# hby1320/pytorch_object_detection

Measured on AMD Instinct MI355X. Metric: images/sec HISFCOS-R50 640x640 inference, higher is better.
Workload: dtype f32

## Files before the change

pytorch_object_detection_amd/csrc/fd_conv_b2b.hip:

```cpp
#include "fd_conv_common.h"

struct B2BArgs {
    const float* x; const float* res; float* y; float* z;
    const float* scale1; const float* shift1; const float* scale2; const float* shift2;
    int x_cs, x_co, res_cs, res_co, y_cs, y_co, z_cs, z_co;
    int M, KT1, NT1, N2, act1, act2;
    unsigned x_bytes, y_bytes, z_bytes, res_bytes;
};

template <int TM, int TN2>
__global__ __launch_bounds__(64, 2) void conv1x1_b2b_kernel(B2BArgs a, const float* __restrict__ wf1_, const float* __restrict__ wf2_) {
    extern __shared__ __attribute__((aligned(16))) char smem[];
    float* As = reinterpret_cast<float*>(smem);
    float* A2 = As + 32 * TM * 32;
    constexpr int NL = 4 * TM;
    const int lane = threadIdx.x, l31 = lane & 31, lh = lane >> 5;
    const int m0 = blockIdx.x * 32 * TM;

    constexpr unsigned OOB = 0xC0000000u;
    const __amdgpu_buffer_rsrc_t xrsrc = __builtin_amdgcn_make_buffer_rsrc((void*)a.x, (short)0, (int)a.x_bytes, 0x00020000);
    const int lrow = lane >> 3, chunk = lane & 7;
    unsigned a_off[NL];
#pragma unroll
    for (int i = 0; i < NL; ++i) {
        const int m = m0 + lrow + 8 * i;
        a_off[i] = (m < a.M) ? ((unsigned)m * (unsigned)a.x_cs + (unsigned)(a.x_co + chunk * 4)) * 4u : OOB;
    }
    const float4* __restrict__ wf1 = reinterpret_cast<const float4*>(wf1_) + lane;
    const float4* __restrict__ wf2 = reinterpret_cast<const float4*>(wf2_) + lane;
    const int KT1 = a.KT1, KT2 = 2 * a.NT1;

    float4 ra[NL];
    auto load_a = [&](int kt) {
        const unsigned kb = (unsigned)kt * 128u;
#pragma unroll
        for (int i = 0; i < NL; ++i)
            ra[i] = __builtin_bit_cast(float4, __builtin_amdgcn_raw_buffer_load_b128(xrsrc, (int)(a_off[i] + kb), 0, 0));
    };
    auto store_a = [&]() {
#pragma unroll
        for (int i = 0; i < NL; ++i) *reinterpret_cast<float4*>(As + lds_off(lrow + 8 * i, chunk)) = ra[i];
    };

    f32x16 acc2[TM][TN2];
#pragma unroll
    for (int i = 0; i < TM; ++i)
#pragma unroll
        for (int j = 0; j < TN2; ++j)
#pragma unroll
            for (int e = 0; e < 16; ++e) acc2[i][j][e] = 0.f;

    const int c4 = (lane & 7) * 4, prow = lane >> 3;
    float* stage = As;
    const __amdgpu_buffer_rsrc_t yrsrc = __builtin_amdgcn_make_buffer_rsrc((void*)a.y, (short)0, (int)a.y_bytes, 0x00020000);
    const __amdgpu_buffer_rsrc_t zrsrc = __builtin_amdgcn_make_buffer_rsrc((void*)a.z, (short)0, (int)a.z_bytes, 0x00020000);
    const __amdgpu_buffer_rsrc_t rrsrc = __builtin_amdgcn_make_buffer_rsrc((void*)(a.res ? a.res : a.x), (short)0, (int)a.res_bytes, 0x00020000);
    const unsigned y_off = ((unsigned)(m0 + prow) * (unsigned)a.y_cs + (unsigned)(a.y_co + c4)) * 4u;
    const unsigned z_off = ((unsigned)(m0 + prow) * (unsigned)a.z_cs + (unsigned)(a.z_co + c4)) * 4u;
    const unsigned r_off = ((unsigned)(m0 + prow) * (unsigned)a.res_cs + (unsigned)(a.res_co + c4)) * 4u;

    for (int n1t = 0; n1t < a.NT1; ++n1t) {
        f32x16 acc1[TM][2];
#pragma unroll
        for (int i = 0; i < TM; ++i)
#pragma unroll
            for (int j = 0; j < 2; ++j)
#pragma unroll
                for (int e = 0; e < 16; ++e) acc1[i][j][e] = 0.f;
        float4 fb[2][2];
        const float4* __restrict__ w1t = wf1 + (size_t)n1t * KT1 * 512;
        load_a(0);
#pragma unroll
        for (int j = 0; j < 2; ++j)
#pragma unroll
            for (int s = 0; s < 2; ++s) fb[j][s] = w1t[(j * 4 + s) * 64];
        for (int kt = 0; kt < KT1; ++kt) {
            store_a();
            __builtin_amdgcn_sched_barrier(0);
            if (kt + 1 < KT1) load_a(kt + 1);
            __builtin_amdgcn_sched_barrier(0);
            wave_lds_sync();
            const float4* __restrict__ wc_ = w1t + (size_t)kt * 512;
            const float4* __restrict__ wn_ = w1t + (size_t)min(kt + 1, KT1 - 1) * 512;
            __builtin_amdgcn_s_setprio(1);
#pragma unroll
            for (int s = 0; s < 4; ++s) {
                float4 fa[TM];
#pragma unroll
                for (int i = 0; i < TM; ++i) fa[i] = *reinterpret_cast<const float4*>(As + lds_off(i * 32 + l31, 2 * s + lh));
#pragma unroll
                for (int i = 0; i < TM; ++i)
#pragma unroll
                    for (int j = 0; j < 2; ++j) {
                        acc1[i][j] = __builtin_amdgcn_mfma_f32_32x32x2f32(fa[i].x, fb[j][s & 1].x, acc1[i][j], 0, 0, 0);
                        acc1[i][j] = __builtin_amdgcn_mfma_f32_32x32x2f32(fa[i].y, fb[j][s & 1].y, acc1[i][j], 0, 0, 0);
                        acc1[i][j] = __builtin_amdgcn_mfma_f32_32x32x2f32(fa[i].z, fb[j][s & 1].z, acc1[i][j], 0, 0, 0);
                        acc1[i][j] = __builtin_amdgcn_mfma_f32_32x32x2f32(fa[i].w, fb[j][s & 1].w, acc1[i][j], 0, 0, 0);
                    }
#pragma unroll
                for (int j = 0; j < 2; ++j) fb[j][s & 1] = s < 2 ? wc_[(j * 4 + s + 2) * 64] : wn_[(j * 4 + s - 2) * 64];
                __builtin_amdgcn_sched_barrier(0);
            }
            __builtin_amdgcn_s_setprio(0);
            wave_lds_sync();
        }

#pragma unroll
        for (int j = 0; j < 2; ++j) {
            const int nb = n1t * 64 + 32 * j;
            const float sc = a.scale1 ? a.scale1[nb + l31] : 1.0f, sf = a.shift1 ? a.shift1[nb + l31] : 0.0f;
            float4 fb2[TN2][2];
            const int kt2 = 2 * n1t + j;
            auto w2at = [&](int jj, int s) { return wf2[((size_t)((jj >> 1) * KT2 + kt2) * 8 + (jj & 1) * 4 + s) * 64]; };
#pragma unroll
            for (int jj = 0; jj < TN2; ++jj)
#pragma unroll
                for (int s = 0; s < 2; ++s) fb2[jj][s] = w2at(jj, s);
#pragma unroll
            for (int i = 0; i < TM; ++i) {
                float4 rr[4];
#pragma unroll
                for (int p = 0; p < 4; ++p)
                    rr[p] = __builtin_bit_cast(float4, __builtin_amdgcn_raw_buffer_load_b128(rrsrc, (int)r_off, ((32 * i + 8 * p) * a.res_cs + nb) * 4, 0));
#pragma unroll
                for (int e = 0; e < 16; ++e) stage[((e & 3) + 8 * (e >> 2) + 4 * lh) * 32 + l31] = acc1[i][j][e] * sc + sf;
                wave_lds_sync();
#pragma unroll
                for (int p = 0; p < 4; ++p) {
                    float4 v = *reinterpret_cast<const float4*>(stage + (prow + 8 * p) * 32 + c4);
                    const float4 r = rr[p];
                    v.x += r.x; v.y += r.y; v.z += r.z; v.w += r.w;
                    if (a.act1 == FD_ACT_RELU) {
                        v.x = fmaxf(v.x, 0.f); v.y = fmaxf(v.y, 0.f); v.z = fmaxf(v.z, 0.f); v.w = fmaxf(v.w, 0.f);
                    } else if (a.act1 == FD_ACT_SILU) {
                        v.x = fd_act(v.x, FD_ACT_SILU, 0.f); v.y = fd_act(v.y, FD_ACT_SILU, 0.f); v.z = fd_act(v.z, FD_ACT_SILU, 0.f); v.w = fd_act(v.w, FD_ACT_SILU, 0.f);
                    }
                    __builtin_amdgcn_raw_buffer_store_b128(__builtin_bit_cast(f32x4, v), yrsrc, (int)y_off, ((32 * i + 8 * p) * a.y_cs + nb) * 4, 0);
                    *reinterpret_cast<float4*>(A2 + lds_off(32 * i + prow + 8 * p, lane & 7)) = v;
                }
                wave_lds_sync();
            }
            __builtin_amdgcn_s_setprio(1);
#pragma unroll
            for (int s = 0; s < 4; ++s) {
                float4 fa[TM];
#pragma unroll
                for (int i = 0; i < TM; ++i) fa[i] = *reinterpret_cast<const float4*>(A2 + lds_off(i * 32 + l31, 2 * s + lh));
#pragma unroll
                for (int i = 0; i < TM; ++i)
#pragma unroll
                    for (int jj = 0; jj < TN2; ++jj) {
                        acc2[i][jj] = __builtin_amdgcn_mfma_f32_32x32x2f32(fa[i].x, fb2[jj][s & 1].x, acc2[i][jj], 0, 0, 0);
                        acc2[i][jj] = __builtin_amdgcn_mfma_f32_32x32x2f32(fa[i].y, fb2[jj][s & 1].y, acc2[i][jj], 0, 0, 0);
                        acc2[i][jj] = __builtin_amdgcn_mfma_f32_32x32x2f32(fa[i].z, fb2[jj][s & 1].z, acc2[i][jj], 0, 0, 0);
                        acc2[i][jj] = __builtin_amdgcn_mfma_f32_32x32x2f32(fa[i].w, fb2[jj][s & 1].w, acc2[i][jj], 0, 0, 0);
                    }
                if (s < 2) {
#pragma unroll
                    for (int jj = 0; jj < TN2; ++jj) fb2[jj][s & 1] = w2at(jj, s + 2);
                }
                __builtin_amdgcn_sched_barrier(0);
            }
            __builtin_amdgcn_s_setprio(0);
            wave_lds_sync();
        }
    }

#pragma unroll
    for (int jj = 0; jj < TN2; ++jj) {
        const int nb = 32 * jj;
        if (nb >= a.N2) break;
        const float sc = a.scale2 ? a.scale2[nb + l31] : 1.0f, sf = a.shift2 ? a.shift2[nb + l31] : 0.0f;
#pragma unroll
        for (int i = 0; i < TM; ++i) {
#pragma unroll
            for (int e = 0; e < 16; ++e) stage[((e & 3) + 8 * (e >> 2) + 4 * lh) * 32 + l31] = acc2[i][jj][e] * sc + sf;
            wave_lds_sync();
#pragma unroll
            for (int p = 0; p < 4; ++p) {
                float4 v = *reinterpret_cast<const float4*>(stage + (prow + 8 * p) * 32 + c4);
                if (a.act2 == FD_ACT_RELU) {
                    v.x = fmaxf(v.x, 0.f); v.y = fmaxf(v.y, 0.f); v.z = fmaxf(v.z, 0.f); v.w = fmaxf(v.w, 0.f);
                } else if (a.act2 == FD_ACT_SILU) {
                    v.x = fd_act(v.x, FD_ACT_SILU, 0.f); v.y = fd_act(v.y, FD_ACT_SILU, 0.f); v.z = fd_act(v.z, FD_ACT_SILU, 0.f); v.w = fd_act(v.w, FD_ACT_SILU, 0.f);
                }
                __builtin_amdgcn_raw_buffer_store_b128(__builtin_bit_cast(f32x4, v), zrsrc, (int)z_off, ((32 * i + 8 * p) * a.z_cs + nb) * 4, 0);
            }
            wave_lds_sync();
        }
    }
}

extern "C" int32_t fd_conv1x1_b2b_f32(const fd_b2b_params* p, fd_stream_t stream_) {
    hipStream_t stream = (hipStream_t)stream_;
    FD_REQUIRE(p && p->x && p->w1_frag && p->w2_frag && p->y && p->z, FD_E_INVAL, "fd_conv1x1_b2b: null pointer");
    FD_REQUIRE(p->rows >= 1 && p->K1 >= 32 && p->K1 % 32 == 0 && p->N1 >= 64 && p->N1 % 64 == 0 && (p->N2 == 64 || p->N2 == 128), FD_E_UNSUPPORTED,
               "fd_conv1x1_b2b: needs K1 %% 32 == 0, N1 %% 64 == 0, N2 in {64, 128} (got %d -> %d -> %d)", p->K1, p->N1, p->N2);
    FD_REQUIRE(p->x_cs % 4 == 0 && p->x_co % 4 == 0 && p->x_cs >= p->x_co + p->K1 && p->y_cs % 4 == 0 && p->y_co % 4 == 0 && p->y_cs >= p->y_co + p->N1 &&
                   p->z_cs % 4 == 0 && p->z_co % 4 == 0 && p->z_cs >= p->z_co + p->N2 &&
                   (!p->res || (p->res_cs % 4 == 0 && p->res_co % 4 == 0 && p->res_cs >= p->res_co + p->N1)),
               FD_E_INVAL, "fd_conv1x1_b2b: channel views must be 4-aligned and in range");
    FD_REQUIRE((((uintptr_t)p->x | (uintptr_t)p->y | (uintptr_t)p->z | (uintptr_t)p->res | (uintptr_t)p->w1_frag | (uintptr_t)p->w2_frag) & 15) == 0, FD_E_INVAL,
               "fd_conv1x1_b2b: pointers must be 16-byte aligned");
    auto act_ok = [](int a_) { return a_ == FD_ACT_NONE || a_ == FD_ACT_RELU || a_ == FD_ACT_SILU; };
    FD_REQUIRE(act_ok(p->act1) && act_ok(p->act2), FD_E_UNSUPPORTED, "fd_conv1x1_b2b: activations none / ReLU / SiLU");
    const long xb = (long)p->rows * p->x_cs * 4;
    FD_REQUIRE(xb < 0xC0000000L - 65536 && (long)p->rows * p->y_cs * 4 < 0xC0000000L && (long)p->rows * p->z_cs * 4 < 0xC0000000L &&
                   (!p->res || (long)p->rows * p->res_cs * 4 < 0xC0000000L), FD_E_UNSUPPORTED, "fd_conv1x1_b2b: a view's buffer exceeds 3 GiB");
    B2BArgs a;
    a.x = p->x; a.res = p->res; a.y = p->y; a.z = p->z;
    a.scale1 = p->scale1; a.shift1 = p->shift1; a.scale2 = p->scale2; a.shift2 = p->shift2;
    a.x_cs = p->x_cs; a.x_co = p->x_co; a.res_cs = p->res_cs; a.res_co = p->res_co; a.y_cs = p->y_cs; a.y_co = p->y_co; a.z_cs = p->z_cs; a.z_co = p->z_co;
    a.M = (int)p->rows; a.KT1 = p->K1 / 32; a.NT1 = p->N1 / 64; a.N2 = p->N2; a.act1 = p->act1; a.act2 = p->act2;
    a.x_bytes = (unsigned)xb;
    a.y_bytes = (unsigned)((long)p->rows * p->y_cs * 4); a.z_bytes = (unsigned)((long)p->rows * p->z_cs * 4);
    a.res_bytes = p->res ? (unsigned)((long)p->rows * p->res_cs * 4) : 0u;
    if (p->N2 == 64) {
        const unsigned blocks = (unsigned)((p->rows + 63) / 64);
        hipLaunchKernelGGL((conv1x1_b2b_kernel<2, 2>), dim3(blocks), dim3(64), 2 * 64 * 32 * 4, stream, a, p->w1_frag, p->w2_frag);
    } else {
        const unsigned blocks = (unsigned)((p->rows + 31) / 32);
        hipLaunchKernelGGL((conv1x1_b2b_kernel<1, 4>), dim3(blocks), dim3(64), 2 * 32 * 32 * 4, stream, a, p->w1_frag, p->w2_frag);
    }
    FD_CHECK_LAUNCH("fd_conv1x1_b2b_f32");
    return FD_OK;
}
```

Measured before the change: 1472.

## Prefetch residual and next-tile loads across b2b conv phases, simplify offsets

Restructures the fused back-to-back 1x1 conv kernel so the residual tile is loaded during the last K iteration of the first GEMM and the next N1 tile's A/weight head is prefetched during the second GEMM, reusing the A staging registers. Scale/shift loads are hoisted out of the epilogue, and the per-row offset arrays are replaced by a single base offset plus a scalar stride, dropping the per-row bounds masking. A host check on stride×rows is added to keep the buffer offsets in range, and optional compile-time timing instrumentation is added. The goal is to hide global load latency between phases and cut register pressure. The trade-off is that out-of-range rows now rely on the buffer size limit rather than explicit masking.

```diff
diff --git a/pytorch_object_detection_amd/csrc/fd_conv_b2b.hip b/pytorch_object_detection_amd/csrc/fd_conv_b2b.hip
--- a/pytorch_object_detection_amd/csrc/fd_conv_b2b.hip
+++ b/pytorch_object_detection_amd/csrc/fd_conv_b2b.hip
@@ -1,4 +1,9 @@
 #include "fd_conv_common.h"
+#ifdef FD_B2B_TIMING
+#include <cstdio>
+#include <cstdlib>
+#include <vector>
+#endif
 
 struct B2BArgs {
     const float* x; const float* res; float* y; float* z;
@@ -6,36 +11,49 @@
     int x_cs, x_co, res_cs, res_co, y_cs, y_co, z_cs, z_co;
     int M, KT1, NT1, N2, act1, act2;
     unsigned x_bytes, y_bytes, z_bytes, res_bytes;
+    long long* ts;
 };
+#ifdef FD_B2B_TIMING
+#define B2B_TS(k) do { __builtin_amdgcn_sched_barrier(0); const long long n_ = wall_clock64(); b2b_acc[k] += n_ - b2b_last; b2b_last = n_; \
+        __builtin_amdgcn_sched_barrier(0); } while (0)
+#define B2B_USE(x) asm volatile("" :: "v"(x))
+#else
+#define B2B_TS(k) do { } while (0)
+#define B2B_USE(x) do { } while (0)
+#endif
 
 template <int TM, int TN2>
 __global__ __launch_bounds__(64, 2) void conv1x1_b2b_kernel(B2BArgs a, const float* __restrict__ wf1_, const float* __restrict__ wf2_) {
     extern __shared__ __attribute__((aligned(16))) char smem[];
+#ifdef FD_B2B_TIMING
+    long long b2b_acc[7] = {0, 0, 0, 0, 0, 0, 0};
+    const long long b2b_t0 = wall_clock64();
+    long long b2b_last = b2b_t0;
+    B2B_TS(6); B2B_TS(6);
+    b2b_acc[6] >>= 1;
+#endif
     float* As = reinterpret_cast<float*>(smem);
     float* A2 = As + 32 * TM * 32;
     constexpr int NL = 4 * TM;
     const int lane = threadIdx.x, l31 = lane & 31, lh = lane >> 5;
     const int m0 = blockIdx.x * 32 * TM;
 
-    constexpr unsigned OOB = 0xC0000000u;
     const __amdgpu_buffer_rsrc_t xrsrc = __builtin_amdgcn_make_buffer_rsrc((void*)a.x, (short)0, (int)a.x_bytes, 0x00020000);
     const int lrow = lane >> 3, chunk = lane & 7;
-    unsigned a_off[NL];
-#pragma unroll
-    for (int i = 0; i < NL; ++i) {
-        const int m = m0 + lrow + 8 * i;
-        a_off[i] = (m < a.M) ? ((unsigned)m * (unsigned)a.x_cs + (unsigned)(a.x_co + chunk * 4)) * 4u : OOB;
-    }
+    const unsigned a_off = ((unsigned)(m0 + lrow) * (unsigned)a.x_cs + (unsigned)(a.x_co + chunk * 4)) * 4u;
+    const int xstep8 = a.x_cs * 32;
     const float4* __restrict__ wf1 = reinterpret_cast<const float4*>(wf1_) + lane;
     const float4* __restrict__ wf2 = reinterpret_cast<const float4*>(wf2_) + lane;
     const int KT1 = a.KT1, KT2 = 2 * a.NT1;
 
     float4 ra[NL];
+#define FD_OPAQUE_S(v) asm volatile("" : "+s"(v))
     auto load_a = [&](int kt) {
-        const unsigned kb = (unsigned)kt * 128u;
+        int xs = xstep8;
+        FD_OPAQUE_S(xs);
 #pragma unroll
         for (int i = 0; i < NL; ++i)
-            ra[i] = __builtin_bit_cast(float4, __builtin_amdgcn_raw_buffer_load_b128(xrsrc, (int)(a_off[i] + kb), 0, 0));
+            ra[i] = __builtin_bit_cast(float4, __builtin_amdgcn_raw_buffer_load_b128(xrsrc, (int)(a_off + (unsigned)(i * xs + kt * 128)), 0, 0));
     };
     auto store_a = [&]() {
 #pragma unroll
@@ -58,6 +76,24 @@
     const unsigned y_off = ((unsigned)(m0 + prow) * (unsigned)a.y_cs + (unsigned)(a.y_co + c4)) * 4u;
     const unsigned z_off = ((unsigned)(m0 + prow) * (unsigned)a.z_cs + (unsigned)(a.z_co + c4)) * 4u;
     const unsigned r_off = ((unsigned)(m0 + prow) * (unsigned)a.res_cs + (unsigned)(a.res_co + c4)) * 4u;
+    const int ystep8 = a.y_cs * 32, zstep8 = a.z_cs * 32, rstep8 = a.res_cs * 32;
+    auto load_res = [&](int n1t, int j) {
+        int rs = rstep8;
+        FD_OPAQUE_S(rs);
+#pragma unroll
+        for (int i = 0; i < NL; ++i)
+            ra[i] = __builtin_bit_cast(float4, __builtin_amdgcn_raw_buffer_load_b128(rrsrc, (int)(r_off + (unsigned)(i * rs + n1t * 256) + 128u * j), 0, 0));
+    };
+    float4 fb[2][2];
+    auto load_tile_head = [&](int n1t) {
+        const float4* __restrict__ w1t = wf1 + (size_t)n1t * KT1 * 512;
+        load_a(0);
+#pragma unroll
+        for (int j = 0; j < 2; ++j)
+#pragma unroll
+            for (int s = 0; s < 2; ++s) fb[j][s] = w1t[(j * 4 + s) * 64];
+    };
+    load_tile_head(0);
 
     for (int n1t = 0; n1t < a.NT1; ++n1t) {
         f32x16 acc1[TM][2];
@@ -67,21 +103,25 @@
             for (int j = 0; j < 2; ++j)
 #pragma unroll
                 for (int e = 0; e < 16; ++e) acc1[i][j][e] = 0.f;
-        float4 fb[2][2];
         const float4* __restrict__ w1t = wf1 + (size_t)n1t * KT1 * 512;
-        load_a(0);
-#pragma unroll
-        for (int j = 0; j < 2; ++j)
-#pragma unroll
-            for (int s = 0; s < 2; ++s) fb[j][s] = w1t[(j * 4 + s) * 64];
-        for (int kt = 0; kt < KT1; ++kt) {
+        float sc1[2], sf1[2];
+        auto ktile = [&](int kt, auto last_c) {
+            constexpr bool LAST = decltype(last_c)::value;
             store_a();
             __builtin_amdgcn_sched_barrier(0);
-            if (kt + 1 < KT1) load_a(kt + 1);
+            if (kt == 0) {
+#pragma unroll
+                for (int j = 0; j < 2; ++j) {
+                    sc1[j] = a.scale1 ? a.scale1[n1t * 64 + 32 * j + l31] : 1.0f;
+                    sf1[j] = a.shift1 ? a.shift1[n1t * 64 + 32 * j + l31] : 0.0f;
+                }
+            }
+            if constexpr (LAST) load_res(n1t, 0);
+            else load_a(kt + 1);
             __builtin_amdgcn_sched_barrier(0);
             wave_lds_sync();
             const float4* __restrict__ wc_ = w1t + (size_t)kt * 512;
-            const float4* __restrict__ wn_ = w1t + (size_t)min(kt + 1, KT1 - 1) * 512;
+            const float4* __restrict__ wn_ = wc_ + 512;
             __builtin_amdgcn_s_setprio(1);
 #pragma unroll
             for (int s = 0; s < 4; ++s) {
@@ -97,18 +137,22 @@
                         acc1[i][j] = __builtin_amdgcn_mfma_f32_32x32x2f32(fa[i].z, fb[j][s & 1].z, acc1[i][j], 0, 0, 0);
                         acc1[i][j] = __builtin_amdgcn_mfma_f32_32x32x2f32(fa[i].w, fb[j][s & 1].w, acc1[i][j], 0, 0, 0);
                     }
-#pragma unroll
-                for (int j = 0; j < 2; ++j) fb[j][s & 1] = s < 2 ? wc_[(j * 4 + s + 2) * 64] : wn_[(j * 4 + s - 2) * 64];
+                if (s < 2 || !LAST) {
+#pragma unroll
+                    for (int j = 0; j < 2; ++j) fb[j][s & 1] = s < 2 ? wc_[(j * 4 + s + 2) * 64] : wn_[(j * 4 + s - 2) * 64];
+                }
                 __builtin_amdgcn_sched_barrier(0);
             }
             __builtin_amdgcn_s_setprio(0);
             wave_lds_sync();
-        }
+        };
+        for (int kt = 0; kt + 1 < KT1; ++kt) ktile(kt, std::false_type{});
+        ktile(KT1 - 1, std::true_type{});
+        B2B_TS(0);
 
 #pragma unroll
         for (int j = 0; j < 2; ++j) {
-            const int nb = n1t * 64 + 32 * j;
-            const float sc = a.scale1 ? a.scale1[nb + l31] : 1.0f, sf = a.shift1 ? a.shift1[nb + l31] : 0.0f;
+            const float sc = sc1[j], sf = sf1[j];
             float4 fb2[TN2][2];
             const int kt2 = 2 * n1t + j;
             auto w2at = [&](int jj, int s) { return wf2[((size_t)((jj >> 1) * KT2 + kt2) * 8 + (jj & 1) * 4 + s) * 64]; };
@@ -118,28 +162,39 @@
                 for (int s = 0; s < 2; ++s) fb2[jj][s] = w2at(jj, s);
 #pragma unroll
             for (int i = 0; i < TM; ++i) {
-                float4 rr[4];
-#pragma unroll
-                for (int p = 0; p < 4; ++p)
-                    rr[p] = __builtin_bit_cast(float4, __builtin_amdgcn_raw_buffer_load_b128(rrsrc, (int)r_off, ((32 * i + 8 * p) * a.res_cs + nb) * 4, 0));
 #pragma unroll
                 for (int e = 0; e < 16; ++e) stage[((e & 3) + 8 * (e >> 2) + 4 * lh) * 32 + l31] = acc1[i][j][e] * sc + sf;
+                int ys = ystep8;
+                FD_OPAQUE_S(ys);
                 wave_lds_sync();
 #pragma unroll
                 for (int p = 0; p < 4; ++p) {
                     float4 v = *reinterpret_cast<const float4*>(stage + (prow + 8 * p) * 32 + c4);
-                    const float4 r = rr[p];
+                    const float4 r = ra[4 * i + p];
+                    if (p == 0) { B2B_TS(1); B2B_USE(r.x); B2B_TS(i == 0 ? 2 : 3); }
                     v.x += r.x; v.y += r.y; v.z += r.z; v.w += r.w;
                     if (a.act1 == FD_ACT_RELU) {
                         v.x = fmaxf(v.x, 0.f); v.y = fmaxf(v.y, 0.f); v.z = fmaxf(v.z, 0.f); v.w = fmaxf(v.w, 0.f);
                     } else if (a.act1 == FD_ACT_SILU) {
                         v.x = fd_act(v.x, FD_ACT_SILU, 0.f); v.y = fd_act(v.y, FD_ACT_SILU, 0.f); v.z = fd_act(v.z, FD_ACT_SILU, 0.f); v.w = fd_act(v.w, FD_ACT_SILU, 0.f);
                     }
-                    __builtin_amdgcn_raw_buffer_store_b128(__builtin_bit_cast(f32x4, v), yrsrc, (int)y_off, ((32 * i + 8 * p) * a.y_cs + nb) * 4, 0);
+                    __builtin_amdgcn_raw_buffer_store_b128(__builtin_bit_cast(f32x4, v), yrsrc, (int)(y_off + (unsigned)((4 * i + p) * ys + n1t * 256) + 128u * j), 0, 0);
                     *reinterpret_cast<float4*>(A2 + lds_off(32 * i + prow + 8 * p, lane & 7)) = v;
                 }
                 wave_lds_sync();
             }
+            __builtin_amdgcn_sched_barrier(0);
+            if (j == 0) load_res(n1t, 1);
+            else if (n1t + 1 < a.NT1) load_tile_head(n1t + 1);
+            else {
+#pragma unroll
+                for (int jj = 0; jj < TN2; ++jj) {
+                    ra[jj].x = a.scale2 ? a.scale2[32 * jj + l31] : 1.0f;
+                    ra[jj].y = a.shift2 ? a.shift2[32 * jj + l31] : 0.0f;
+                }
+            }
+            __builtin_amdgcn_sched_barrier(0);
+            B2B_TS(1);
             __builtin_amdgcn_s_setprio(1);
 #pragma unroll
             for (int s = 0; s < 4; ++s) {
@@ -163,6 +218,7 @@
             }
             __builtin_amdgcn_s_setprio(0);
             wave_lds_sync();
+            B2B_TS(4);
         }
     }
 
@@ -170,11 +226,13 @@
     for (int jj = 0; jj < TN2; ++jj) {
         const int nb = 32 * jj;
         if (nb >= a.N2) break;
-        const float sc = a.scale2 ? a.scale2[nb + l31] : 1.0f, sf = a.shift2 ? a.shift2[nb + l31] : 0.0f;
+        const float sc = ra[jj].x, sf = ra[jj].y;
 #pragma unroll
         for (int i = 0; i < TM; ++i) {
 #pragma unroll
             for (int e = 0; e < 16; ++e) stage[((e & 3) + 8 * (e >> 2) + 4 * lh) * 32 + l31] = acc2[i][jj][e] * sc + sf;
+            int zs = zstep8;
+            FD_OPAQUE_S(zs);
             wave_lds_sync();
 #pragma unroll
             for (int p = 0; p < 4; ++p) {
@@ -184,11 +242,20 @@
                 } else if (a.act2 == FD_ACT_SILU) {
                     v.x = fd_act(v.x, FD_ACT_SILU, 0.f); v.y = fd_act(v.y, FD_ACT_SILU, 0.f); v.z = fd_act(v.z, FD_ACT_SILU, 0.f); v.w = fd_act(v.w, FD_ACT_SILU, 0.f);
                 }
-                __builtin_amdgcn_raw_buffer_store_b128(__builtin_bit_cast(f32x4, v), zrsrc, (int)z_off, ((32 * i + 8 * p) * a.z_cs + nb) * 4, 0);
+                __builtin_amdgcn_raw_buffer_store_b128(__builtin_bit_cast(f32x4, v), zrsrc, (int)(z_off + (unsigned)((4 * i + p) * zs) + 128u * jj), 0, 0);
             }
             wave_lds_sync();
         }
     }
+#ifdef FD_B2B_TIMING
+    B2B_TS(5);
+    if (a.ts && lane == 0) {
+        long long* r_ = a.ts + (size_t)blockIdx.x * 8;
+#pragma unroll
+        for (int k = 0; k < 7; ++k) r_[k] = b2b_acc[k];
+        r_[7] = b2b_last - b2b_t0;
+    }
+#endif
 }
 
 extern "C" int32_t fd_conv1x1_b2b_f32(const fd_b2b_params* p, fd_stream_t stream_) {
@@ -207,6 +274,8 @@
     const long xb = (long)p->rows * p->x_cs * 4;
     FD_REQUIRE(xb < 0xC0000000L - 65536 && (long)p->rows * p->y_cs * 4 < 0xC0000000L && (long)p->rows * p->z_cs * 4 < 0xC0000000L &&
                    (!p->res || (long)p->rows * p->res_cs * 4 < 0xC0000000L), FD_E_UNSUPPORTED, "fd_conv1x1_b2b: a view's buffer exceeds 3 GiB");
+    const long cs_max = std::max(std::max((long)p->x_cs, (long)p->y_cs), std::max((long)p->z_cs, p->res ? (long)p->res_cs : 0L));
+    FD_REQUIRE((p->rows + 64) * cs_max * 4 + 65536 < 0x100000000L, FD_E_UNSUPPORTED, "fd_conv1x1_b2b: a view's row stride is too large for its row count");
     B2BArgs a;
     a.x = p->x; a.res = p->res; a.y = p->y; a.z = p->z;
     a.scale1 = p->scale1; a.shift1 = p->shift1; a.scale2 = p->scale2; a.shift2 = p->shift2;
@@ -215,6 +284,39 @@
     a.x_bytes = (unsigned)xb;
     a.y_bytes = (unsigned)((long)p->rows * p->y_cs * 4); a.z_bytes = (unsigned)((long)p->rows * p->z_cs * 4);
     a.res_bytes = p->res ? (unsigned)((long)p->rows * p->res_cs * 4) : 0u;
+    a.ts = nullptr;
+#ifdef FD_B2B_TIMING
+    static const char* ts_path = getenv("FD_B2B_TS");
+    static long long* ts_dev = nullptr;
+    const size_t ts_n = (size_t)((p->rows + (p->N2 == 64 ? 63 : 31)) / (p->N2 == 64 ? 64 : 32)) * 8;
+    if (ts_path && ts_n <= (size_t)(1 << 16) * 8) {
+        if (!ts_dev) (void)hipMalloc((void**)&ts_dev, (size_t)(1 << 16) * 8 * sizeof(long long));
+        if (ts_dev) { a.ts = ts_dev; (void)hipMemsetAsync(ts_dev, 0, ts_n * sizeof(long long), stream); }
+    }
+    struct TsDump {
+        const char* path; size_t n; hipStream_t st; const B2BArgs& a; const fd_b2b_params* p;
+        ~TsDump() {
+            if (!path || !a.ts) return;
+            (void)hipStreamSynchronize(st);
+            std::vector<long long> h(n);
+            (void)hipMemcpy(h.data(), a.ts, n * sizeof(long long), hipMemcpyDeviceToHost);
+            double m[8] = {0, 0, 0, 0, 0, 0, 0, 0}, totmax = 0; size_t live = 0;
+            for (size_t b = 0; b < n / 8; ++b) {
+                if (!h[b * 8 + 7]) continue;
+                for (int k = 0; k < 8; ++k) m[k] += (double)h[b * 8 + k];
+                if ((double)h[b * 8 + 7] > totmax) totmax = (double)h[b * 8 + 7];
+                ++live;
+            }
+            if (FILE* f = fopen(path, "a")) {
+                const double u = 0.01 / (live ? live : 1);
+                fprintf(f, "b2bts K1 %d N1 %d N2 %d rows %ld res %d waves %zu | per-wave us: phase1 %.2f epilogue1 %.2f wait_res_first %.2f wait_res_later %.2f phase2 %.2f "
+                        "epilogue2 %.2f | total %.2f max %.2f | one stamp %.3f\n", p->K1, p->N1, p->N2, (long)p->rows, p->res ? 1 : 0, live, m[0] * u, m[1] * u, m[2] * u,
+                        m[3] * u, m[4] * u, m[5] * u, m[7] * u, totmax * 0.01, m[6] * u);
+                fclose(f);
+            }
+        }
+    } ts_dump{ts_path, ts_n, stream, a, p};
+#endif
     if (p->N2 == 64) {
         const unsigned blocks = (unsigned)((p->rows + 63) / 64);
         hipLaunchKernelGGL((conv1x1_b2b_kernel<2, 2>), dim3(blocks), dim3(64), 2 * 64 * 32 * 4, stream, a, p->w1_frag, p->w2_frag);
```

Result: no change. 1476, median of 6 (+0.2%).
